# knight46/Quantum_compute_DFT

Measured on AMD Instinct MI355X. Metric: grid_points_per_sec, higher is better.
Workload: dtype f64; 1 GPU; benzene_gga_def2svp: DFT_ComputeXC (GGA) nao=114 ngrid=143556 per GPU, synthetic AO/grid (SURVEY 8(d) recipe), inputs resident in HBM; functional=GGA, nao=114, nocc=21, ngrid_per_gpu=143556, entry_point=DFT_ComputeXC (the reference ABI: full density matrix)

## Files before the change

### include/dft_solver.h

```cpp
#ifndef QCDFT_AMD_DFT_SOLVER_H
#define QCDFT_AMD_DFT_SOLVER_H

#ifdef __cplusplus
extern "C" {
#endif

typedef struct XCSolver XCSolver;

enum SolverType { SOLVER_LDA = 0, SOLVER_GGA = 1, SOLVER_B3LYP = 2,
                  SOLVER_MIX = 3  };

enum XCComponent { XC_SLATER_X = 0, XC_VWN5_C, XC_VWN_RPA_C, XC_PW92_C,
                   XC_PBE_X, XC_PBE_C, XC_B88_X, XC_LYP_C, XC_NCOMP };


XCSolver *DFT_CreateSolver(int type);

void DFT_DestroySolver(XCSolver *solver);

double DFT_ComputeXC(XCSolver *solver, int ngrid, int nao,
                     unsigned long long d_dm_ptr,
                     unsigned long long d_ao_ptr,
                     unsigned long long d_ao_grad_ptr,
                     unsigned long long d_weights_ptr,
// ... 108 lines not shown
int DFT_PointCoulombSetStream(void *handle, unsigned long long hip_stream);
const char *DFT_PointCoulombLastError(void *handle);
void DFT_PointCoulombClose(void *handle);

void *DFT_ScfTailOpen(int nao, int nocc, unsigned long long d_hcore, unsigned long long d_overlap, unsigned long long d_basis,
                      unsigned long long d_fock_out, unsigned long long d_mo_energy);
int DFT_ScfTailSetStream(void *handle, unsigned long long hip_stream);
int DFT_ScfTailStep(void *handle, int rotate, double c_hf, double tol, double canon_tol, int max_inner, int slot, int nhist,
                    const int *hist, const double *coef, unsigned long long d_J, unsigned long long d_K,
                    unsigned long long d_vraw, unsigned long long d_dm, unsigned long long d_cocc, unsigned long long d_exc);
int DFT_ScfTailFinish(void *handle, double c_hf, unsigned long long d_J, unsigned long long d_K, unsigned long long d_dm,
                      unsigned long long d_cocc);
int DFT_ScfTailMore(void *handle, int nsteps, unsigned long long d_J, unsigned long long d_K, unsigned long long d_dm,
                    unsigned long long d_cocc, unsigned long long d_exc);
int DFT_ScfTailSetStepsHint(void *handle, int nsteps);
int DFT_ScfTailWait(void *handle, double *out8);
int DFT_ScfTailGram(void *handle, double *host_out64);
int DFT_ScfTailStamps(void *handle, long long *host_out16);
const char *DFT_ScfTailLastError(void *handle);
void DFT_ScfTailClose(void *handle);

int DFT_SetOption(XCSolver *solver, const char *key, double value);

int DFT_SetStream(XCSolver *solver, unsigned long long hip_stream);

const char *DFT_GetLastError(XCSolver *solver);

int DFT_GetTimings(XCSolver *solver, double *ms, const char **names, int max_entries);

#ifdef __cplusplus
}
#endif
#endif
```

### quantum_compute_dft_amd/build.py

```python
import contextlib
import fcntl
import hashlib
import json
import os
import re
import shutil
import subprocess

PKG_DIR = os.path.dirname(os.path.abspath(__file__))
CSRC = os.path.join(PKG_DIR, "csrc")
LIB_DIR = os.path.join(PKG_DIR, "lib")
LIB_PATH = os.path.join(LIB_DIR, "libdft.so")
STAMP_PATH = LIB_PATH + ".srchash"
SOURCES = ["dft_api.hip", "xc_occ.hip", "eri_cols.hip", "scf_tail.hip", "xc_tiny.hip", "point_coulomb.hip"]
HEADERS = ["xc_functionals.hpp", "xc_kernels.hpp", "xc_ws_kernels.hpp", "xc_big_kernels.hpp",
           "xc_occ_kernels.hpp", "xc_occ_launch.hpp", "xc_tiny_kernels.hpp", "xc_tiny_launch.hpp", "jk_kernels.hpp", "ao_kernels.hpp", "cd_kernels.hpp", "device_util.hpp", "md_device.hpp",
           os.path.join("..", "..", "include", "dft_solver.h")]
FLAGS = ["--offload-arch=gfx950", "-O3", "-std=c++17", "-fPIC",
         "-mllvm", "-amdgpu-mfma-vgpr-form", "-Wall", "-Wno-unused-function"]
EXTRA_FLAGS = {"xc_tiny.hip": ["-mllvm", "-disable-machine-licm"]}
RESOURCES_PATH = LIB_PATH + ".resources.json"

VALIDATION_KERNELS = ("k_rho_mfma", "k_vxc_mfma", "k_rho_valu", "k_vxc_valu")
SPILL_ALLOW = {
    "void qcdft::k_vxc_ws<8, true, false, false>": (8, "one dword (the thread index) stored before and reloaded after the step loop, "
                                                       "never inside it (ISA checked); the 8-byte-load GGA variant for odd nao / "
                                                       "unaligned planes at nao 113-128 only"),
}


def parse_resource_usage(text):
    out = {}
    for blk in re.split(r"remark: Function Name: ", text)[1:]:
        name = blk.split()[0]
        def g(key):
            m = re.search(key + r": (\d+)", blk)
            return int(m.group(1)) if m else 0
        out[name] = {"vgprs": g(r"  VGPRs"), "agprs": g("AGPRs"), "sgprs": g(r"  SGPRs"), "vgpr_spill": g("VGPRs Spill"),
                     "sgpr_spill": g("SGPRs Spill"), "scratch": g(r"ScratchSize \[bytes/lane\]"),
                     "occupancy": g(r"Occupancy \[waves/SIMD\]"), "lds": g(r"LDS Size \[bytes/block\]")}
    return out


def check_spills(res):
    bad = []
    for name, r in sorted(res.items()):
        if not (r["vgpr_spill"] or r["scratch"]):
            continue
# ... 105 lines not shown
```

### quantum_compute_dft_amd/csrc/dft_api.hip

```cpp
#include <hip/hip_runtime.h>

#include <cmath>
#include <cstdarg>
#include <cstdio>
#include <cstdint>
#include <cstdlib>
#include <cstring>
#include <algorithm>
#include <limits>
#include <string>
#include <type_traits>
#include <vector>

#include "../../include/dft_solver.h"
#include "ao_kernels.hpp"
#include "jk_kernels.hpp"
#include "cd_kernels.hpp"
#include "xc_big_kernels.hpp"
#include "xc_ws_kernels.hpp"
#include "xc_kernels.hpp"
#include "xc_occ_launch.hpp"
#include "xc_tiny_launch.hpp"

using namespace qcdft;
// ... 20 lines not shown
    unsigned long stamp = 0;
};

}

struct XCSolver {
    int type = 0;
    bool needs_grad = false;
    xc::MixWeights mix = {};
    hipStream_t stream = nullptr;
    bool device_ok = false;
    int device = 0;
    int num_cu = 256;
    int quirks = 1;
    int path = 0;
    int profile = 0;
    int ksplit = 0;
    int ao_pt = 0;
    int fuse_finish = 0;
    int sweep_order = 2;
    int tiny = -1;
    int occ = 0;
    int used_occ = 0;
    int eri_sym = 0;
    int graph = -1;
    std::vector<SweepGraph> graphs;
    hipStream_t cap_stream = nullptr;
    unsigned long graph_clock = 0, graph_gen = 0;
    DevBuf dsym, rho, sigma, grad, coef, partial, slabs, exc, jpart, kpart, shells, msym, cdy, cdc, cdv, ao_ws, vtmp, occ_cp, occ_dm;
    int spin_wait = 1;
    int strict_sync = 0;
    double *h_exc = nullptr;
    double *h_exc_dev = nullptr;
    std::string last_error;
    std::vector<Timing> timings;
    size_t n_timed = 0;
    std::vector<unsigned char> shell_blob;
};

namespace {

void set_error(XCSolver *s, const char *fmt, ...)
{
    char buf[512];
    va_list ap;
    va_start(ap, fmt);
    vsnprintf(buf, sizeof buf, fmt, ap);
    va_end(ap);
    fprintf(stderr, "libdft: %s\n", buf);
    if (s) s->last_error = buf;
}

bool hip_ok(XCSolver *s, hipError_t e, const char *what)
{
    if (e == hipSuccess) return true;
    set_error(s, "%s failed: %s", what, hipGetErrorString(e));
// ... 73 lines not shown

template <int NT = 1, class F>
void with_nt(int nt, F &&f)
{
    if constexpr (NT < 8) {
        if (nt != NT) return with_nt<NT + 1>(nt, f);
    }
    f(std::integral_constant<int, NT>{});
}

template <class F>
void with_bool(bool b, F &&f)
{
    if (b) f(std::true_type{});
    else   f(std::false_type{});
}

bool xc_sweep(XCSolver *s, long ngrid, int nao, const double *dm, const double *ao,
              const double *ao_grad, const double *w, double *vxc, bool want_host_exc,
              const double *cocc = nullptr, int nocc = 0, double *exc_out = nullptr)
{
    s->last_error.clear();
    s->n_timed = 0;
    if (!s->device_ok) {
        set_error(s, "no usable HIP device");
        return false;
    }
    if (ngrid <= 0 || nao <= 0) {
        set_error(s, "bad sizes ngrid=%ld nao=%d", ngrid, nao);
        return false;
    }
    const bool gga = s->needs_grad;
    if (gga && !ao_grad) {
        set_error(s, "ao_grad pointer is null for a gradient-corrected functional");
        return false;
    }
    if (!dm && !cocc) {
        set_error(s, "neither a density matrix nor occupied orbitals were given");
        return false;
    }
    if (cocc && nocc <= 0) {
        set_error(s, "occupied orbitals given with nocc=%d", nocc);
        return false;
    }
    const bool tiny = s->path == 0 && s->tiny != 0 && s->type != SOLVER_MIX && nao <= TINY_MAX_NAO && (double)ngrid * nao * 8.0 < 4294967296.0 &&
                      (s->tiny > 0 || tiny_pays(s->num_cu, s->type == SOLVER_LDA ? 0 : s->type == SOLVER_GGA ? 1 : 2, nao, ngrid));
// ... 93 lines not shown
                    hipLaunchKernelGGL((k_rho_ws<NT, G, V>), dim3((unsigned)nslab), dim3(WS_THREADS), 0, st, ngrid, nao, ao, gx, gy, gz, dm, rho, grad, sigma, s->sweep_order & 1);
                }); });
            else if (big)
                with_bool(vec16, [&](auto V) {
                    hipLaunchKernelGGL((k_rho_big64<G, V>), dim3((unsigned)((ngrid + R6_BM - 1) / R6_BM)), dim3(256), 0, st, ngrid, nao, NP, ao, gx, gy, gz, Dp, rho, grad, sigma);
                });
            else if (s->path != 1)
                hipLaunchKernelGGL(k_rho_mfma<G>, dim3((unsigned)((ngrid + 63) / 64)), dim3(256), 0, st, ngrid, nao, NP, ao, gx, gy, gz, Dp, rho, grad, sigma);
            else
                hipLaunchKernelGGL(k_rho_valu<G>, dim3((unsigned)((ngrid + 3) / 4)), dim3(256), 0, st, ngrid, nao, NP, ao, gx, gy, gz, Dp, rho, grad, sigma);
        });
    }
    if (!tiny) {
        ScopedTimer t(s, "xc_points");
        dim3 g((unsigned)nxb);
        if (s->type == SOLVER_LDA)      hipLaunchKernelGGL(k_xc_points<0>, g, dim3(256), 0, st, ngrid, rho, sigma, grad, w, coef, partial, s->quirks);
        else if (s->type == SOLVER_GGA) hipLaunchKernelGGL(k_xc_points<1>, g, dim3(256), 0, st, ngrid, rho, sigma, grad, w, coef, partial, s->quirks);
        else if (s->type == SOLVER_B3LYP) hipLaunchKernelGGL(k_xc_points<2>, g, dim3(256), 0, st, ngrid, rho, sigma, grad, w, coef, partial, s->quirks);
        else if (gga)                   hipLaunchKernelGGL(k_xc_points_mix<true>, g, dim3(256), 0, st, ngrid, rho, sigma, grad, w, coef, partial, s->quirks, s->mix);
        else                            hipLaunchKernelGGL(k_xc_points_mix<false>, g, dim3(256), 0, st, ngrid, rho, sigma, grad, w, coef, partial, s->quirks, s->mix);
    }
    if (!tiny) {
        ScopedTimer t(s, "vxc");
        auto launch = [&](auto G, auto S) {
            if (fast)
                with_bool(vec16, [&](auto V) { with_nt(ntv, [&](auto NT) {
                    hipLaunchKernelGGL((k_vxc_ws<NT, G, V, S>), dim3((unsigned)nslab), dim3(WS_THREADS), 0, st, ngrid, nao, ao, gx, gy, gz, coef, slabs, (s->sweep_order >> 1) & 1);
                }); });
            else if (big)
                with_bool(vec16, [&](auto V) {
                    hipLaunchKernelGGL((k_vxc_big<G, V>), dim3((unsigned)(nslab * npair)), dim3(BG_THREADS), 0, st, ngrid, nao, chunk, nB, npair, ao, gx, gy, gz, coef, slabs);
                });
            else if (s->path != 1)
                hipLaunchKernelGGL(k_vxc_mfma<G>, dim3((unsigned)nslab, nblk, nblk), dim3(256), 0, st, ngrid, nao, chunk, ao, gx, gy, gz, coef, slabs);
            else
                hipLaunchKernelGGL(k_vxc_valu<G>, dim3((unsigned)nslab), dim3(256), 0, st, ngrid, nao, chunk, ao, gx, gy, gz, coef, slabs);
        };
        switch (s->type) {
        case SOLVER_LDA: launch(std::false_type{}, std::false_type{}); break;
        case SOLVER_GGA: launch(std::true_type{}, std::false_type{}); break;
        case SOLVER_MIX:
            if (gga) launch(std::true_type{}, std::false_type{});
            else     launch(std::false_type{}, std::false_type{});
            break;
        default:         launch(std::true_type{}, std::true_type{}); break;
        }
    }
    {
        ScopedTimer t(s, "reduce_vxc");
        dim3 g((unsigned)(((size_t)nao * nao + 31) / 32));
        const bool b3 = s->type == SOLVER_B3LYP;
        if (b3 && big) {
            if (!reserve(s, s->msym, sizeof(double) * (size_t)nao * nao, "hipMalloc(M)")) return false;
            double *M = (double *)s->msym.p;
            hipLaunchKernelGGL(k_reduce_slabs8<false>, g, dim3(256), 0, st, nao, nslab, slabs, M);
            const int nt = (nao + 31) / 32;
            hipLaunchKernelGGL(k_symmetrize, dim3((unsigned)(nt * (nt + 1) / 2)), dim3(256), 0, st, nao, M, vxc);
        } else if (b3 && !fast) {
            hipLaunchKernelGGL(k_reduce_slabs8<true>, g, dim3(256), 0, st, nao, nslab, slabs, vxc);
        } else if (s->fuse_finish) {
            hipLaunchKernelGGL((k_reduce_slabs8<false, true>), g, dim3(256), 0, st, nao, nslab, slabs, vxc, nxb, partial, exc,
                               want_host_exc ? s->h_exc_dev : nullptr);
            return hip_ok(s, hipGetLastError(), "XC sweep launch");
        } else {
            hipLaunchKernelGGL((k_reduce_slabs8<false, true>), g, dim3(256), 0, st, nao, nslab, slabs, vxc, nxb, partial, exc, (double *)nullptr);
            if (want_host_exc && s->h_exc_dev) hipLaunchKernelGGL(k_publish_exc, dim3(1), dim3(1), 0, st, exc, s->h_exc_dev);
            return hip_ok(s, hipGetLastError(), "XC sweep launch");
        }
        hipLaunchKernelGGL(k_finish_exc, dim3(1), dim3(256), 0, st, nxb, partial, exc, want_host_exc ? s->h_exc_dev : nullptr);
    }
    return hip_ok(s, hipGetLastError(), "XC sweep launch");
}

void jk(XCSolver *s, int nao, const double *eri, const double *dm, double *J, double *K, int i0 = 0, int ni = -1)
{
    s->last_error.clear();
    if (!s->device_ok) { set_error(s, "no usable HIP device"); return; }
    if (nao <= 0 || nao > JK_COLS) { set_error(s, "dense-ERI J/K needs 1 <= nao <= %d (got %d)", JK_COLS, nao); return; }
    if (ni < 0) ni = nao;
    if (i0 < 0 || ni <= 0 || i0 + ni > nao) { set_error(s, "dense-ERI J/K: bad row range [%d, %d) of %d", i0, i0 + ni, nao); return; }
    if (!J && !K) return;
    const int n = nao;
    const size_t N2 = (size_t)n * n;
    const int KB = std::max(1, std::min(n, JK_COLS / n));
    const int ncb = (n + KB - 1) / KB;
    if (J && !K && s->eri_sym == 2 && i0 == 0 && ni == n && n >= 48) {
        const size_t NPK = (size_t)n * (n + 1) / 2;
        const int nchunk = (int)((NPK + JS8_RC - 1) / JS8_RC);
        int cpt = 4;
// ... 245 lines not shown

void launch_ao(XCSolver *s, const AoTable &t, long ngrid, int nao, const double *coords, double *ao, double *ao_grad)
{
    const bool vec = t.even_blocks && (nao % 2 == 0) && ((uintptr_t)ao % 16 == 0) && ((uintptr_t)ao_grad % 16 == 0);
    const int ao_pt = s->ao_pt ? s->ao_pt : ((ao_grad ? 4 : 1) * 16 * (t.maxcol | 1) * 8 > 53 * 1024 ? 8 : 16);
    launch_eval_ao(s->stream, ngrid, nao, t.nchunk, t.maxcol, vec, ao_pt, s->num_cu, t.nshell, t.nprim, t.sh, t.exp, t.coef, t.chunks, t.order,
                   coords, ao, ao_grad);
}

__global__ void k_accumulate_chunk(long n2, int add, const double *__restrict__ vc, const double *__restrict__ ec,
                                   double *__restrict__ v, double *__restrict__ e)
{
    const long i = (long)blockIdx.x * 256 + threadIdx.x;
    if (i < n2) v[i] = add ? v[i] + vc[i] : vc[i];
    if (i == 0) *e = add ? *e + *ec : *ec;
}

}

extern "C" {

int DFT_GetVersion(void) { return 5; }

static XCSolver *create_solver(int type, const double *mix)
{
    XCSolver *s = new (std::nothrow) XCSolver();
    if (!s) return nullptr;
    s->type = type;
    s->needs_grad = type != SOLVER_LDA;
    if (mix) {
        s->needs_grad = false;
        for (int k = 0; k < XC_NCOMP; ++k) {
            s->mix.c[k] = mix[k];
            if (k >= XC_PBE_X && mix[k] != 0.0) s->needs_grad = true;
        }
    }
    int ndev = 0;
    if (hipGetDeviceCount(&ndev) == hipSuccess && ndev > 0) {
        int dev = 0;
        hipDeviceProp_t prop;
        if (hipGetDevice(&dev) == hipSuccess && hipGetDeviceProperties(&prop, dev) == hipSuccess) {
            s->device_ok = true;
            s->device = dev;
            s->num_cu = prop.multiProcessorCount > 0 ? prop.multiProcessorCount : 256;
        }
        if (s->device_ok) {
            if (hipHostMalloc((void **)&s->h_exc, sizeof(double), hipHostMallocMapped | hipHostMallocCoherent) != hipSuccess ||
                hipHostGetDevicePointer((void **)&s->h_exc_dev, s->h_exc, 0) != hipSuccess) {
                (void)hipGetLastError();
                s->h_exc = nullptr;
                s->h_exc_dev = nullptr;
            }
        }
    } else {
        (void)hipGetLastError();
        s->last_error = "no usable HIP device";
    }
    return s;
}

XCSolver *DFT_CreateSolver(int type)
{
    if (type != SOLVER_LDA && type != SOLVER_GGA && type != SOLVER_B3LYP) return nullptr;
    return create_solver(type, nullptr);
}

XCSolver *DFT_CreateSolverMix(const double *weights, int ncomp)
{
    if (!weights || ncomp != XC_NCOMP) return nullptr;
    bool any = false;
    for (int k = 0; k < XC_NCOMP; ++k) {
        if (!std::isfinite(weights[k])) return nullptr;
        any = any || weights[k] != 0.0;
    }
    if (!any) return nullptr;
// ... 10 lines not shown
    case SOLVER_B3LYP:
        weights_out[XC_SLATER_X] = 0.80; weights_out[XC_B88_X] = 0.72; weights_out[XC_VWN_RPA_C] = 0.19; weights_out[XC_LYP_C] = 0.81;
        break;
    default:
        for (int k = 0; k < XC_NCOMP; ++k) weights_out[k] = s->mix.c[k];
    }
    return 0;
}

void DFT_DestroySolver(XCSolver *s)
{
    if (!s) return;
    if (s->device_ok) {
        DeviceGuard dg(s);
        (void)hipStreamSynchronize(s->stream);
        drop_graphs(s);
        if (s->cap_stream) (void)hipStreamDestroy(s->cap_stream);
        DevBuf *bufs[] = {&s->dsym, &s->rho, &s->sigma, &s->grad, &s->coef, &s->partial,
                          &s->slabs, &s->exc, &s->jpart, &s->kpart, &s->shells, &s->msym,
                          &s->cdy, &s->cdc, &s->cdv, &s->ao_ws, &s->vtmp, &s->occ_cp, &s->occ_dm};
        for (DevBuf *b : bufs)
            if (b->p) (void)hipFree(b->p);
        if (s->h_exc) (void)hipHostFree(s->h_exc);
        for (Timing &t : s->timings) {
            (void)hipEventDestroy(t.t0);
            (void)hipEventDestroy(t.t1);
        }
    }
    delete s;
}

constexpr double GRAPH_AUTO_ELEMS = 2.0e6;

struct SweepArgs {
    long ngrid;
    int nao, nocc;
    const double *dm, *ao, *grad, *w;
    double *vxc;
    const double *cocc;
};

static SweepGraph *find_sweep(XCSolver *s, const SweepArgs &a)
{
    for (SweepGraph &g : s->graphs)
        if (g.ngrid == a.ngrid && g.nao == a.nao && g.nocc == a.nocc && g.dm == a.dm && g.ao == a.ao && g.grad == a.grad &&
            g.w == a.w && g.vxc == a.vxc && g.cocc == a.cocc)
            return &g;
    return nullptr;
}

static bool record_sweep(XCSolver *s, const SweepArgs &a)
{
    if (!s->cap_stream && hipStreamCreateWithFlags(&s->cap_stream, hipStreamNonBlocking) != hipSuccess) {
        (void)hipGetLastError();
        return false;
    }
    const unsigned long gen = s->graph_gen;
    if (hipStreamBeginCapture(s->cap_stream, hipStreamCaptureModeThreadLocal) != hipSuccess) {
        (void)hipGetLastError();
        return false;
    }
    hipStream_t user = s->stream;
    s->stream = s->cap_stream;
    const bool ok = xc_sweep(s, a.ngrid, a.nao, a.dm, a.ao, a.grad, a.w, a.vxc, true, a.cocc, a.nocc);
    s->stream = user;
    hipGraph_t graph = nullptr;
    const hipError_t e = hipStreamEndCapture(s->cap_stream, &graph);
    hipGraphExec_t exec = nullptr;
    const bool good = ok && e == hipSuccess && graph && gen == s->graph_gen &&
                      hipGraphInstantiate(&exec, graph, nullptr, nullptr, 0) == hipSuccess;
    if (graph) (void)hipGraphDestroy(graph);
    if (!good) (void)hipGetLastError();
    SweepGraph *g = gen == s->graph_gen ? find_sweep(s, a) : nullptr;
    if (!g) {
        if (exec) (void)hipGraphExecDestroy(exec);
        return false;
    }
    g->exec = good ? exec : nullptr;
    g->bad = !good;
    return good;
}

static bool replay_sweep(XCSolver *s, const SweepArgs &a)
{
    SweepGraph *g = find_sweep(s, a);
    if (!g || g->bad) return false;
    if (!g->exec && !record_sweep(s, a)) return false;
// ... 26 lines not shown
        s->graphs.erase(s->graphs.begin() + (long)old);
    }
    SweepGraph g;
    g.ngrid = a.ngrid; g.nao = a.nao; g.nocc = a.nocc;
    g.dm = a.dm; g.ao = a.ao; g.grad = a.grad; g.w = a.w; g.vxc = a.vxc; g.cocc = a.cocc;
    g.seen = 1;
    g.stamp = ++s->graph_clock;
    s->graphs.push_back(g);
}

static double xc_call_sync(XCSolver *s, long long ngrid, int nao, unsigned long long d_dm,
                           unsigned long long d_ao, unsigned long long d_ao_grad,
                           unsigned long long d_w, unsigned long long d_vxc,
                           unsigned long long d_cocc, int nocc)
{
    if (!s) return 0.0;
    DeviceGuard dg(s);
    const double nan = std::numeric_limits<double>::quiet_NaN();
    if (s->h_exc) *s->h_exc = nan;
    const SweepArgs a{(long)ngrid, nao, nocc, (const double *)d_dm, (const double *)d_ao, (const double *)d_ao_grad,
                      (const double *)d_w, (double *)d_vxc, (const double *)d_cocc};
    const bool graphed = !s->profile && s->h_exc_dev && ngrid > 0 && nao > 0 &&
                         (s->graph > 0 || (s->graph < 0 && (double)ngrid * nao <= GRAPH_AUTO_ELEMS));
    if (!(graphed && replay_sweep(s, a)) &&
        !xc_sweep(s, a.ngrid, nao, a.dm, a.ao, a.grad, a.w, a.vxc, true, a.cocc, nocc))
        return nan;
    if (graphed) note_sweep(s, a);
    if (s->h_exc_dev) {
        volatile double *hx = s->h_exc;
        if (s->spin_wait) {
            for (unsigned spins = 1; std::isnan(*hx); ++spins) {
                if ((spins & 0xFFF) == 0 && hipStreamQuery(s->stream) != hipErrorNotReady) break;
                __builtin_ia32_pause();
            }
            if (s->strict_sync || std::isnan(*hx)) {
                hipError_t q;
                while ((q = hipStreamQuery(s->stream)) == hipErrorNotReady) __builtin_ia32_pause();
                if (!hip_ok(s, q, "XC sweep")) return nan;
            }
        } else if (!hip_ok(s, hipStreamSynchronize(s->stream), "synchronise")) {
            return nan;
        }
        const double out = *hx;
        if (std::isnan(out)) set_error(s, "Exc is NaN after the sweep completed (non-finite inputs, or the finishing kernel did not run)");
        return out;
    }
    double out = nan;
    if (!hip_ok(s, hipMemcpyAsync(&out, s->exc.p, sizeof(double), hipMemcpyDeviceToHost, s->stream), "copy Exc") ||
        !hip_ok(s, hipStreamSynchronize(s->stream), "synchronise"))
        return nan;
    if (std::isnan(out)) set_error(s, "Exc is NaN after the sweep completed (non-finite inputs)");
    return out;
}
// ... 143 lines not shown
        hipLaunchKernelGGL(k_accumulate_chunk, dim3(nb), dim3(256), 0, s->stream, (long)nao * nao, g0 == 0 ? 0 : 1, vt,
                           (const double *)s->exc.p, (double *)d_vxc, eacc);
    }
    if (d_exc && !hip_ok(s, hipMemcpyAsync((void *)d_exc, eacc, sizeof(double), hipMemcpyDeviceToDevice, s->stream), "copy Exc"))
        return -1;
    return hip_ok(s, hipGetLastError(), "direct XC sweep launch") ? 0 : -1;
}

int DFT_SetOption(XCSolver *s, const char *key, double value)
{
    if (!s || !key) return -1;
    if (strcmp(key, "profile") && strcmp(key, "spin_wait") && strcmp(key, "strict_sync")) {
        DeviceGuard dg(s);
        drop_graphs(s);
    }
    if (!strcmp(key, "eri_symmetric")) { s->eri_sym = value == 2.0 ? 2 : value != 0.0; return 0; }
    if (!strcmp(key, "graph")) { s->graph = value > 0.0 ? 1 : value < 0.0 ? -1 : 0; return 0; }
    if (!strcmp(key, "quirks")) { s->quirks = value != 0.0; return 0; }
    if (!strcmp(key, "path")) { s->path = (int)value; return 0; }
    if (!strcmp(key, "profile")) { s->profile = value != 0.0; return 0; }
    if (!strcmp(key, "spin_wait")) { s->spin_wait = value != 0.0; return 0; }
    if (!strcmp(key, "strict_sync")) { s->strict_sync = value != 0.0; return 0; }
    if (!strcmp(key, "fuse_finish")) { s->fuse_finish = value != 0.0; return 0; }
    if (!strcmp(key, "sweep_order")) { s->sweep_order = (int)value & 3; return 0; }
    if (!strcmp(key, "occ")) { s->occ = value == 1.0 ? 1 : value == 2.0 ? 2 : 0; return 0; }
    if (!strcmp(key, "tiny")) { s->tiny = value > 0.0 ? 1 : value < 0.0 ? -1 : 0; return 0; }
    if (!strcmp(key, "ao_pt")) { s->ao_pt = value == 16.0 ? 16 : value == 8.0 ? 8 : 0; return 0; }
    if (!strcmp(key, "ksplit")) { s->ksplit = value > 0 ? (int)value : 0; return 0; }
    return -1;
}

int DFT_SetStream(XCSolver *s, unsigned long long hip_stream)
{
    if (!s) return -1;
    DeviceGuard dg(s);
    if (s->device_ok) (void)hipStreamSynchronize(s->stream);
    s->stream = (hipStream_t)hip_stream;
    return 0;
}

const char *DFT_GetLastError(XCSolver *s)
{
    return s ? s->last_error.c_str() : "";
}

int DFT_GetTimings(XCSolver *s, double *ms, const char **names, int max_entries)
{
    if (!s || !s->device_ok) return 0;
    DeviceGuard dg(s);
    (void)hipStreamSynchronize(s->stream);
    int n = 0;
    for (size_t i = 0; i < s->n_timed && n < max_entries; ++i, ++n) {
// ... 10 lines not shown
```

### quantum_compute_dft_amd/csrc/xc_ws_kernels.hpp

```cpp
#pragma once
#include <hip/hip_runtime.h>
#include "xc_kernels.hpp"

namespace qcdft {

#ifdef QCDFT_STAMPS
__device__ unsigned long long g_stamps[256 * 8 * 4];
#define QCDFT_T(var) unsigned long long var = __builtin_amdgcn_s_memtime()
#define QCDFT_ACC(slot, a, b) st_acc[slot] += (b) - (a)
#else
#define QCDFT_T(var)
#define QCDFT_ACC(slot, a, b)
#endif

constexpr int WS_ROWS = 16;
constexpr int WS_THREADS = 512;
constexpr int WS_RING = 4;
constexpr int WS_OT = 16;

template <int NT> struct WsCfg {
    static constexpr int NCOL = 16 * NT;
    static constexpr int JN = (NT + 1) / 2;
    static constexpr int LDA = NCOL + 2;
    static constexpr int LDX = ((NCOL + 31) / 32) * 32 + 16;
};

__device__ __forceinline__ unsigned ws_tile(unsigned ntile, unsigned b, unsigned s, unsigned nwg, int rev)
{
    const unsigned t = b + s * nwg;
    return rev ? ntile - 1u - t : t;
}

template <int NT, bool GRAD, bool VEC, bool SYM>
__global__ __launch_bounds__(WS_THREADS, 2) void k_vxc_ws(long ngrid, int nao,
                                                          const double *__restrict__ ao,
                                                          const double *__restrict__ gx,
                                                          const double *__restrict__ gy,
                                                          const double *__restrict__ gz,
                                                          const double *__restrict__ coef,
                                                          double *__restrict__ slabs, int rev)
{
    using C = WsCfg<NT>;
    constexpr int TILE = WS_ROWS * C::LDX;
    constexpr int NTW = (NT + 1) / 2;
    __shared__ double ring[2 * WS_RING * TILE];
    double *const Ps = ring, *const Qs = ring + WS_RING * TILE;

    const int tid = threadIdx.x;
    const int wave = __builtin_amdgcn_readfirstlane(tid >> 6);
    const long ntile = (ngrid + WS_ROWS - 1) / WS_ROWS;
    const long nloc = (ntile > (long)blockIdx.x) ? (ntile - blockIdx.x + gridDim.x - 1) / gridDim.x : 0;
    const long nstep = nloc + 2;

    if (wave < 4) {
        const int lane = tid & 63, li = lane & 15, lk = lane >> 4;
        const int wa = wave >> 1, wb = wave & 1;
        const int na = (NT - wa + 1) / 2, nb = (NT - wb + 1) / 2;
        d4 acc[NTW][NTW];
#pragma unroll
        for (int i = 0; i < NTW; ++i)
#pragma unroll
            for (int j = 0; j < NTW; ++j) acc[i][j] = (d4){0.0, 0.0, 0.0, 0.0};

#ifdef QCDFT_STAMPS
        unsigned long long st_acc[4] = {0, 0, 0, 0};
#endif
        const int fo = lk * C::LDX + li;
        double af[NTW], bf[NTW];
        auto load_frags = [&](int slot, int ks, double (&a_)[NTW], double (&b_)[NTW]) {
            const double *P = Ps + slot * TILE + fo + 4 * ks * C::LDX;
            const double *Q = Qs + slot * TILE + fo + 4 * ks * C::LDX;
#pragma unroll
            for (int i = 0; i < NTW; ++i) {
                a_[i] = Q[16 * min(wa + 2 * i, NT - 1)];
                b_[i] = P[16 * min(wb + 2 * i, NT - 1)];
            }
        };
// ... 39 lines not shown
                for (int j = 0; j < NTW; ++j) {
                    if (i >= na || j >= nb) continue;
                    const int b = 16 * (wb + 2 * j) + li;
#pragma unroll
                    for (int r = 0; r < 4; ++r) {
                        const int a = 16 * (wa + 2 * i) + lk + 4 * r;
                        if (a < nao && b < nao) slab[(size_t)a * nao + b] = acc[i][j][r];
                    }
                }
        } else {
            constexpr int LDM = C::NCOL + 1;
            static_assert(LDM * C::NCOL <= 2 * WS_RING * TILE, "M tile must fit in the ring");
            double *M = ring;
#pragma unroll
            for (int i = 0; i < NTW; ++i)
#pragma unroll
                for (int j = 0; j < NTW; ++j) {
                    if (i >= na || j >= nb) continue;
                    const int b = 16 * (wb + 2 * j) + li;
#pragma unroll
                    for (int r = 0; r < 4; ++r) M[(16 * (wa + 2 * i) + lk + 4 * r) * LDM + b] = acc[i][j][r];
                }
        }
    } else {
        __builtin_amdgcn_s_setprio(3);
        const int lt = tid - 256, row = lt >> 4, seg = lt & 15;
        const double *c0 = coef, *c1 = coef + (size_t)ngrid, *c2 = coef + 2 * (size_t)ngrid,
                     *c3 = coef + 3 * (size_t)ngrid;
        double p0[2][2 * C::JN], p1[2][2 * C::JN], p2[2][2 * C::JN], p3[2][2 * C::JN];
        double k0[2], k1[2], k2[2], k3[2];

        const long plane = ngrid * (long)nao;
        const unsigned voff = (unsigned)(row * nao + 2 * seg) * 8u, koff = (unsigned)row * 8u;
        const unsigned tile_b = (unsigned)(WS_ROWS * nao) * 8u, ktile_b = WS_ROWS * 8u;
        const unsigned plane_b = (unsigned)(plane * 8), coef_b = (unsigned)(ngrid * 8);
        const __amdgpu_buffer_rsrc_t r0 = plane_rsrc(ao, plane), r1 = plane_rsrc(GRAD ? gx : ao, plane),
                                     r2 = plane_rsrc(GRAD ? gy : ao, plane), r3 = plane_rsrc(GRAD ? gz : ao, plane),
                                     q0 = plane_rsrc(c0, ngrid), q1 = plane_rsrc(GRAD ? c1 : c0, ngrid),
                                     q2 = plane_rsrc(GRAD ? c2 : c0, ngrid), q3 = plane_rsrc(GRAD ? c3 : c0, ngrid);
        auto issue = [&](int set, unsigned s) {
            const bool live = s < (unsigned)nloc;
            const unsigned t = ws_tile((unsigned)ntile, blockIdx.x, s, gridDim.x, rev);
            const unsigned so = live ? t * tile_b : plane_b, ko = live ? t * ktile_b : coef_b;
            k0[set] = buf_load_f64(q0, koff, ko);
            if (GRAD) {
                k1[set] = buf_load_f64(q1, koff, ko);
                k2[set] = buf_load_f64(q2, koff, ko);
// ... 392 lines not shown
```

### quantum_compute_dft_amd/solver.py

```python
import ctypes
import os

from . import functionals
from .build import LIB_PATH

_u64 = ctypes.c_uint64


def default_library_path():
    return LIB_PATH


def load_library(lib_path=None):
    try:
        import torch
    except ImportError:
        pass
    return ctypes.CDLL(os.path.abspath(lib_path or default_library_path()))


def _ptr(a):
    if a is None:
        return 0
    if isinstance(a, int):
# ... 41 lines not shown
                                       _u64, _u64, _u64, _u64, _u64, _u64]
        L.DFT_ComputeXCOcc.restype = ctypes.c_double
        L.DFT_ComputeXCOccAsync.argtypes = [ctypes.c_void_p, ctypes.c_longlong, ctypes.c_int, ctypes.c_int,
                                            _u64, _u64, _u64, _u64, _u64, _u64, _u64]
        L.DFT_ComputeXCOccAsync.restype = ctypes.c_int
        L.DFT_ComputeExchange.argtypes = [ctypes.c_void_p, ctypes.c_int, _u64, _u64, _u64]
        L.DFT_ComputeExchange.restype = None
        L.DFT_ComputeJK.argtypes = [ctypes.c_void_p, ctypes.c_int, _u64, _u64, _u64, _u64]
        L.DFT_ComputeJK.restype = None
        L.DFT_ComputeJKRows.argtypes = [ctypes.c_void_p, ctypes.c_int, ctypes.c_int, ctypes.c_int, _u64, _u64, _u64, _u64]
        L.DFT_ComputeJKRows.restype = ctypes.c_int
        L.DFT_ComputeJKFactorized.argtypes = [ctypes.c_void_p, ctypes.c_int, ctypes.c_int, ctypes.c_int,
                                              _u64, _u64, _u64, _u64, _u64]
        L.DFT_ComputeJKFactorized.restype = ctypes.c_int
        dp, ip = ctypes.POINTER(ctypes.c_double), ctypes.POINTER(ctypes.c_int)
        L.DFT_EvalAO.argtypes = [ctypes.c_void_p, ctypes.c_longlong, ctypes.c_int, ctypes.c_int,
                                 dp, ip, ip, ip, ip, dp, dp, ctypes.c_int, _u64, _u64, _u64]
        L.DFT_EvalAO.restype = ctypes.c_int
        L.DFT_ComputeXCDirect.argtypes = [ctypes.c_void_p, ctypes.c_longlong, ctypes.c_int, ctypes.c_int,
                                          dp, ip, ip, ip, ip, dp, dp, ctypes.c_int, _u64, _u64, _u64, _u64, _u64, ctypes.c_longlong]
        L.DFT_ComputeXCDirect.restype = ctypes.c_int
        L.DFT_SetOption.argtypes = [ctypes.c_void_p, ctypes.c_char_p, ctypes.c_double]
        L.DFT_SetOption.restype = ctypes.c_int
        L.DFT_SetStream.argtypes = [ctypes.c_void_p, _u64]
        L.DFT_SetStream.restype = ctypes.c_int
        L.DFT_GetLastError.argtypes = [ctypes.c_void_p]
        L.DFT_GetLastError.restype = ctypes.c_char_p
        L.DFT_GetTimings.argtypes = [ctypes.c_void_p, dp, ctypes.POINTER(ctypes.c_char_p), ctypes.c_int]
        L.DFT_GetTimings.restype = ctypes.c_int
        L.DFT_GetVersion.argtypes = []
        L.DFT_GetVersion.restype = ctypes.c_int
        L.DFT_CreateSolverMix.argtypes = [dp, ctypes.c_int]
        L.DFT_CreateSolverMix.restype = ctypes.c_void_p
        L.DFT_GetMix.argtypes = [ctypes.c_void_p, dp, ctypes.c_int]
        L.DFT_GetMix.restype = ctypes.c_int

        if self.functional.builtin_type is not None:
            self.solver = L.DFT_CreateSolver(self.functional.builtin_type)
        else:
            self.solver = L.DFT_CreateSolverMix((ctypes.c_double * len(self.weights))(*self.weights), len(self.weights))
        if not self.solver:
            raise RuntimeError("Failed to create C++ DFT Solver instance.")

    def __del__(self):
        if hasattr(self, "lib") and hasattr(self, "solver") and self.solver:
            self.lib.DFT_DestroySolver(self.solver)
# ... 69 lines not shown
    def eval_ao(self, shells, d_coords, ngrid, d_ao, d_ao_grad=None):
        keep, args = self._shell_args(shells)
        rc = self.lib.DFT_EvalAO(self.solver, int(ngrid), *args, _u64(_ptr(d_coords)), _u64(_ptr(d_ao)), _u64(_ptr(d_ao_grad)))
        self._check()
        return rc

    def compute_xc_direct(self, shells, ngrid, d_coords, d_weights, d_dm, d_vxc, d_exc, chunk_points=0):
        keep, args = self._shell_args(shells)
        rc = self.lib.DFT_ComputeXCDirect(self.solver, int(ngrid), *args, _u64(_ptr(d_coords)), _u64(_ptr(d_weights)),
                                          _u64(_ptr(d_dm)), _u64(_ptr(d_vxc)), _u64(_ptr(d_exc)), int(chunk_points))
        self._check()
        return rc

    def mix(self):
        out = (ctypes.c_double * len(functionals.COMPONENTS))()
        if self.lib.DFT_GetMix(self.solver, out, len(out)) != 0:
            raise RuntimeError("DFT_GetMix failed")
        return list(out)

    def set_option(self, key, value):
        if self.lib.DFT_SetOption(self.solver, key.encode(), float(value)) != 0:
            raise KeyError(key)

    def set_stream(self, hip_stream):
        self.lib.DFT_SetStream(self.solver, _u64(int(hip_stream)))

    def last_error(self):
        return (self.lib.DFT_GetLastError(self.solver) or b"").decode()

    def timings(self, max_entries=16):
        ms = (ctypes.c_double * max_entries)()
        names = (ctypes.c_char_p * max_entries)()
        n = self.lib.DFT_GetTimings(self.solver, ms, names, max_entries)
        return [(names[i].decode(), ms[i]) for i in range(n)]

    def _check(self):
        err = self.lib.DFT_GetLastError(self.solver)
        if err:
            raise RuntimeError("libdft: " + err.decode())
```

Measured before the change: 650.3 million grid-points/s.

## Add fringe vxc kernel for nao just past 16-multiples and seq-flag host publish

Adds a k_vxc_ws variant for nao with a small remainder over a multiple of 16 (e.g. 114 = 7*16+2). It computes NT-1 full MFMA tiles across three waves and handles the 1-4 leftover rows and columns with scalar FMAs on a fourth wave, avoiding a whole padded 16-wide tile. It also adds an optional host-publish path where the reduce kernel writes exc directly and a stream write of a sequence number signals completion, so the host spins on that counter. The publish path is off by default, and a GetOption query API is added.

```diff
diff --git a/include/dft_solver.h b/include/dft_solver.h
--- a/include/dft_solver.h
+++ b/include/dft_solver.h
@@ -154,6 +154,8 @@
 
 int DFT_SetOption(XCSolver *solver, const char *key, double value);
 
+double DFT_GetOption(XCSolver *solver, const char *key);
+
 int DFT_SetStream(XCSolver *solver, unsigned long long hip_stream);
 
 const char *DFT_GetLastError(XCSolver *solver);
diff --git a/quantum_compute_dft_amd/build.py b/quantum_compute_dft_amd/build.py
--- a/quantum_compute_dft_amd/build.py
+++ b/quantum_compute_dft_amd/build.py
@@ -23,7 +23,7 @@
 
 VALIDATION_KERNELS = ("k_rho_mfma", "k_vxc_mfma", "k_rho_valu", "k_vxc_valu")
 SPILL_ALLOW = {
-    "void qcdft::k_vxc_ws<8, true, false, false>": (8, "one dword (the thread index) stored before and reloaded after the step loop, "
+    "void qcdft::k_vxc_ws<8, true, false, false, false>": (8, "one dword (the thread index) stored before and reloaded after the step loop, "
                                                        "never inside it (ISA checked); the 8-byte-load GGA variant for odd nao / "
                                                        "unaligned planes at nao 113-128 only"),
 }
diff --git a/quantum_compute_dft_amd/csrc/dft_api.hip b/quantum_compute_dft_amd/csrc/dft_api.hip
--- a/quantum_compute_dft_amd/csrc/dft_api.hip
+++ b/quantum_compute_dft_amd/csrc/dft_api.hip
@@ -66,6 +66,9 @@
     int tiny = -1;
     int occ = 0;
     int used_occ = 0;
+    int vxc_fringe = -1;
+    int used_vxc_fringe = 0;
+    int used_publish = 0;
     int eri_sym = 0;
     int graph = -1;
     std::vector<SweepGraph> graphs;
@@ -76,6 +79,12 @@
     int strict_sync = 0;
     double *h_exc = nullptr;
     double *h_exc_dev = nullptr;
+    int publish = -1;
+    bool publish_ok = false;
+    unsigned long long *h_seq = nullptr, *h_seq_dev = nullptr;
+    unsigned long long seq = 0;
+    bool recording = false;
+    int wait_mode = 0;
     std::string last_error;
     std::vector<Timing> timings;
     size_t n_timed = 0;
@@ -195,6 +204,8 @@
 {
     s->last_error.clear();
     s->n_timed = 0;
+    s->wait_mode = 0;
+    s->used_vxc_fringe = 0;
     if (!s->device_ok) {
         set_error(s, "no usable HIP device");
         return false;
@@ -334,9 +345,17 @@
     }
     if (!tiny) {
         ScopedTimer t(s, "vxc");
+        const bool fringe = fast && s->type != SOLVER_B3LYP && s->vxc_fringe != 0 && nao > 16 && nao % 16 >= 1 && nao % 16 <= 4;
+        s->used_vxc_fringe = fringe;
         auto launch = [&](auto G, auto S) {
             if (fast)
                 with_bool(vec16, [&](auto V) { with_nt(ntv, [&](auto NT) {
+                    if constexpr (NT >= 2 && !S) {
+                        if (fringe) {
+                            hipLaunchKernelGGL((k_vxc_ws<NT, G, V, false, true>), dim3((unsigned)nslab), dim3(WS_THREADS), 0, st, ngrid, nao, ao, gx, gy, gz, coef, slabs, (s->sweep_order >> 1) & 1);
+                            return;
+                        }
+                    }
                     hipLaunchKernelGGL((k_vxc_ws<NT, G, V, S>), dim3((unsigned)nslab), dim3(WS_THREADS), 0, st, ngrid, nao, ao, gx, gy, gz, coef, slabs, (s->sweep_order >> 1) & 1);
                 }); });
             else if (big)
@@ -375,8 +394,21 @@
                                want_host_exc ? s->h_exc_dev : nullptr);
             return hip_ok(s, hipGetLastError(), "XC sweep launch");
         } else {
-            hipLaunchKernelGGL((k_reduce_slabs8<false, true>), g, dim3(256), 0, st, nao, nslab, slabs, vxc, nxb, partial, exc, (double *)nullptr);
-            if (want_host_exc && s->h_exc_dev) hipLaunchKernelGGL(k_publish_exc, dim3(1), dim3(1), 0, st, exc, s->h_exc_dev);
+            const bool sw = want_host_exc && s->h_exc_dev && s->publish > 0 && s->publish_ok && !s->recording;
+            hipLaunchKernelGGL((k_reduce_slabs8<false, true>), g, dim3(256), 0, st, nao, nslab, slabs, vxc, nxb, partial, exc,
+                               sw ? s->h_exc_dev : (double *)nullptr);
+            if (sw) {
+                if (hipStreamWriteValue64(st, s->h_seq_dev, s->seq + 1, 0) == hipSuccess) {
+                    ++s->seq;
+                    s->wait_mode = 1;
+                } else {
+                    (void)hipGetLastError();
+                    s->publish_ok = false;
+                    s->wait_mode = 2;
+                }
+            } else if (want_host_exc && s->h_exc_dev) {
+                hipLaunchKernelGGL(k_publish_exc, dim3(1), dim3(1), 0, st, exc, s->h_exc_dev);
+            }
             return hip_ok(s, hipGetLastError(), "XC sweep launch");
         }
         hipLaunchKernelGGL(k_finish_exc, dim3(1), dim3(256), 0, st, nxb, partial, exc, want_host_exc ? s->h_exc_dev : nullptr);
@@ -668,6 +700,25 @@
 
 int DFT_GetVersion(void) { return 5; }
 
+static void probe_publish(XCSolver *s)
+{
+    if (!s->h_exc_dev) return;
+    if (hipHostMalloc((void **)&s->h_seq, sizeof(unsigned long long), hipHostMallocMapped | hipHostMallocCoherent) != hipSuccess ||
+        hipHostGetDevicePointer((void **)&s->h_seq_dev, s->h_seq, 0) != hipSuccess) {
+        (void)hipGetLastError();
+        if (s->h_seq) (void)hipHostFree(s->h_seq);
+        s->h_seq = s->h_seq_dev = nullptr;
+        return;
+    }
+    *s->h_seq = 0;
+    s->seq = 1;
+    if (hipStreamWriteValue64(s->stream, s->h_seq_dev, s->seq, 0) != hipSuccess || hipStreamSynchronize(s->stream) != hipSuccess) {
+        (void)hipGetLastError();
+        return;
+    }
+    s->publish_ok = *(volatile unsigned long long *)s->h_seq == s->seq;
+}
+
 static XCSolver *create_solver(int type, const double *mix)
 {
     XCSolver *s = new (std::nothrow) XCSolver();
@@ -697,6 +748,7 @@
                 s->h_exc = nullptr;
                 s->h_exc_dev = nullptr;
             }
+            probe_publish(s);
         }
     } else {
         (void)hipGetLastError();
@@ -753,6 +805,7 @@
         for (DevBuf *b : bufs)
             if (b->p) (void)hipFree(b->p);
         if (s->h_exc) (void)hipHostFree(s->h_exc);
+        if (s->h_seq) (void)hipHostFree(s->h_seq);
         for (Timing &t : s->timings) {
             (void)hipEventDestroy(t.t0);
             (void)hipEventDestroy(t.t1);
@@ -793,7 +846,9 @@
     }
     hipStream_t user = s->stream;
     s->stream = s->cap_stream;
+    s->recording = true;
     const bool ok = xc_sweep(s, a.ngrid, a.nao, a.dm, a.ao, a.grad, a.w, a.vxc, true, a.cocc, a.nocc);
+    s->recording = false;
     s->stream = user;
     hipGraph_t graph = nullptr;
     const hipError_t e = hipStreamEndCapture(s->cap_stream, &graph);
@@ -866,13 +921,27 @@
                       (const double *)d_w, (double *)d_vxc, (const double *)d_cocc};
     const bool graphed = !s->profile && s->h_exc_dev && ngrid > 0 && nao > 0 &&
                          (s->graph > 0 || (s->graph < 0 && (double)ngrid * nao <= GRAPH_AUTO_ELEMS));
-    if (!(graphed && replay_sweep(s, a)) &&
-        !xc_sweep(s, a.ngrid, nao, a.dm, a.ao, a.grad, a.w, a.vxc, true, a.cocc, nocc))
+    if (graphed && replay_sweep(s, a)) s->wait_mode = 0;
+    else if (!xc_sweep(s, a.ngrid, nao, a.dm, a.ao, a.grad, a.w, a.vxc, true, a.cocc, nocc))
         return nan;
     if (graphed) note_sweep(s, a);
+    s->used_publish = s->wait_mode == 1;
     if (s->h_exc_dev) {
         volatile double *hx = s->h_exc;
-        if (s->spin_wait) {
+        if (s->spin_wait && s->wait_mode == 1) {
+            volatile unsigned long long *hs = s->h_seq;
+            const unsigned long long want = s->seq;
+            for (unsigned spins = 1; *hs != want; ++spins) {
+                if ((spins & 0xFFF) == 0 && hipStreamQuery(s->stream) != hipErrorNotReady) break;
+                __builtin_ia32_pause();
+            }
+            __atomic_thread_fence(__ATOMIC_ACQUIRE);
+            if (s->strict_sync || *hs != want || std::isnan(*hx)) {
+                hipError_t q;
+                while ((q = hipStreamQuery(s->stream)) == hipErrorNotReady) __builtin_ia32_pause();
+                if (!hip_ok(s, q, "XC sweep")) return nan;
+            }
+        } else if (s->spin_wait && s->wait_mode == 0) {
             for (unsigned spins = 1; std::isnan(*hx); ++spins) {
                 if ((spins & 0xFFF) == 0 && hipStreamQuery(s->stream) != hipErrorNotReady) break;
                 __builtin_ia32_pause();
@@ -1062,12 +1131,35 @@
     if (!strcmp(key, "spin_wait")) { s->spin_wait = value != 0.0; return 0; }
     if (!strcmp(key, "strict_sync")) { s->strict_sync = value != 0.0; return 0; }
     if (!strcmp(key, "fuse_finish")) { s->fuse_finish = value != 0.0; return 0; }
+    if (!strcmp(key, "vxc_fringe")) { s->vxc_fringe = value > 0.0 ? 1 : value < 0.0 ? -1 : 0; return 0; }
+    if (!strcmp(key, "publish")) { s->publish = value > 0.0 ? 1 : value < 0.0 ? -1 : 0; return 0; }
     if (!strcmp(key, "sweep_order")) { s->sweep_order = (int)value & 3; return 0; }
     if (!strcmp(key, "occ")) { s->occ = value == 1.0 ? 1 : value == 2.0 ? 2 : 0; return 0; }
     if (!strcmp(key, "tiny")) { s->tiny = value > 0.0 ? 1 : value < 0.0 ? -1 : 0; return 0; }
     if (!strcmp(key, "ao_pt")) { s->ao_pt = value == 16.0 ? 16 : value == 8.0 ? 8 : 0; return 0; }
     if (!strcmp(key, "ksplit")) { s->ksplit = value > 0 ? (int)value : 0; return 0; }
     return -1;
+}
+
+double DFT_GetOption(XCSolver *s, const char *key)
+{
+    const double unknown = std::numeric_limits<double>::quiet_NaN();
+    if (!s || !key) return unknown;
+    if (!strcmp(key, "publish")) return s->publish;
+    if (!strcmp(key, "publish_probe")) return s->publish_ok ? 1.0 : 0.0;
+    if (!strcmp(key, "publish_live")) return s->publish > 0 && s->publish_ok ? 1.0 : 0.0;
+    if (!strcmp(key, "used_publish")) return s->used_publish;
+    if (!strcmp(key, "vxc_fringe")) return s->vxc_fringe;
+    if (!strcmp(key, "used_vxc_fringe")) return s->used_vxc_fringe;
+    if (!strcmp(key, "fuse_finish")) return s->fuse_finish;
+    if (!strcmp(key, "strict_sync")) return s->strict_sync;
+    if (!strcmp(key, "spin_wait")) return s->spin_wait;
+    if (!strcmp(key, "graph")) return s->graph;
+    if (!strcmp(key, "tiny")) return s->tiny;
+    if (!strcmp(key, "sweep_order")) return s->sweep_order;
+    if (!strcmp(key, "path")) return s->path;
+    if (!strcmp(key, "quirks")) return s->quirks;
+    return unknown;
 }
 
 int DFT_SetStream(XCSolver *s, unsigned long long hip_stream)
diff --git a/quantum_compute_dft_amd/csrc/xc_ws_kernels.hpp b/quantum_compute_dft_amd/csrc/xc_ws_kernels.hpp
--- a/quantum_compute_dft_amd/csrc/xc_ws_kernels.hpp
+++ b/quantum_compute_dft_amd/csrc/xc_ws_kernels.hpp
@@ -31,7 +31,122 @@
     return rev ? ntile - 1u - t : t;
 }
 
-template <int NT, bool GRAD, bool VEC, bool SYM>
+template <int NT, int FP>
+__device__ __forceinline__ void vxc_ws_mfma_fringe(const double *Ps, const double *Qs, int tid, int wave, int nao, long nstep,
+                                                   double *__restrict__ slab)
+{
+    using C = WsCfg<NT>;
+    constexpr int NF = NT - 1, F0 = 16 * NF;
+    constexpr int TILE = WS_ROWS * C::LDX;
+    constexpr int NOPP = F0 + 4 > 64 ? 2 : 1;
+    static_assert(NT >= 2 && F0 + 4 <= 128, "one whole tile at least, two opposite indices per lane at most");
+    const int lane = tid & 63, li = lane & 15, lk = lane >> 4;
+    constexpr bool FRW = FP > 0;
+    constexpr int ROWS = FRW ? (NF > 6 ? 1 : 0) : 2, RA = ROWS ? ROWS : 1, NL = FRW ? 2 * FP : 1;
+    const int nr = FRW || NF >= 6 ? ROWS : min(2, max(0, NF - 2 * wave));
+    d4 acc[RA][NF];
+#pragma unroll
+    for (int i = 0; i < RA; ++i)
+#pragma unroll
+        for (int j = 0; j < NF; ++j) acc[i][j] = (d4){0.0, 0.0, 0.0, 0.0};
+    double fa[NL][NOPP], fb[NL][NOPP];
+#pragma unroll
+    for (int f = 0; f < NL; ++f)
+#pragma unroll
+        for (int j = 0; j < NOPP; ++j) { fa[f][j] = 0.0; fb[f][j] = 0.0; }
+    int opp[NOPP];
+#pragma unroll
+    for (int j = 0; j < NOPP; ++j) opp[j] = min(lane + 64 * j, C::NCOL - 1);
+
+    const int fo = lk * C::LDX + li;
+    double af[RA], bf[NF];
+    auto load_frags = [&](int slot, int ks, double (&a_)[RA], double (&b_)[NF]) {
+        if (ROWS == 0) return;
+        const double *P = Ps + slot * TILE + fo + 4 * ks * C::LDX;
+        const double *Q = Qs + slot * TILE + fo + 4 * ks * C::LDX;
+#pragma unroll
+        for (int i = 0; i < RA; ++i) a_[i] = Q[16 * min(2 * wave + i, NF - 1)];
+#pragma unroll
+        for (int j = 0; j < NF; ++j) b_[j] = P[16 * j];
+    };
+    auto fringe_pair = [&](const double *Pr, const double *Qr, const double (&po)[NOPP], const double (&qo)[NOPP], int f) {
+        const double2 pf = *reinterpret_cast<const double2 *>(&Pr[F0 + f]);
+        const double2 qf = *reinterpret_cast<const double2 *>(&Qr[F0 + f]);
+#pragma unroll
+        for (int j = 0; j < NOPP; ++j) {
+            fa[f][j] += qf.x * po[j];
+            fa[f + 1][j] += qf.y * po[j];
+            fb[f][j] += qo[j] * pf.x;
+            fb[f + 1][j] += qo[j] * pf.y;
+        }
+    };
+#pragma unroll
+    for (int i = 0; i < RA; ++i) af[i] = 0.0;
+#pragma unroll
+    for (int j = 0; j < NF; ++j) bf[j] = 0.0;
+    for (long base = 0; base < nstep; base += WS_RING) {
+#pragma unroll
+        for (int u = 0; u < WS_RING; ++u) {
+            const long step = base + u;
+            if (step >= 2 && step < nstep) {
+                if (step == 2) load_frags((u + 2) % WS_RING, 0, af, bf);
+#pragma unroll
+                for (int ks = 0; ks < WS_ROWS / 4; ++ks) {
+                    double an[RA], bn[NF];
+                    if (ks + 1 < WS_ROWS / 4) load_frags((u + 2) % WS_RING, ks + 1, an, bn);
+                    else                      load_frags((u + 3) % WS_RING, 0, an, bn);
+#pragma unroll
+                    for (int i = 0; i < ROWS; ++i)
+                        if (i < nr) {
+#pragma unroll
+                            for (int j = 0; j < NF; ++j) acc[i][j] = mfma_f64(af[i], bf[j], acc[i][j]);
+                        }
+                    if (FRW) {
+#pragma unroll
+                        for (int kk = 0; kk < 4; ++kk) {
+                            const double *Pr = Ps + ((u + 2) % WS_RING) * TILE + (4 * ks + kk) * C::LDX;
+                            const double *Qr = Qs + ((u + 2) % WS_RING) * TILE + (4 * ks + kk) * C::LDX;
+                            double po[NOPP], qo[NOPP];
+#pragma unroll
+                            for (int j = 0; j < NOPP; ++j) { po[j] = Pr[opp[j]]; qo[j] = Qr[opp[j]]; }
+                            fringe_pair(Pr, Qr, po, qo, 0);
+                            if (FP > 1) fringe_pair(Pr, Qr, po, qo, 2);
+                        }
+                    }
+#pragma unroll
+                    for (int i = 0; i < RA; ++i) af[i] = an[i];
+#pragma unroll
+                    for (int j = 0; j < NF; ++j) bf[j] = bn[j];
+                    __builtin_amdgcn_sched_barrier(0);
+                }
+            }
+            __syncthreads();
+        }
+    }
+#pragma unroll
+    for (int i = 0; i < ROWS; ++i) {
+        if (i >= nr) continue;
+#pragma unroll
+        for (int j = 0; j < NF; ++j)
+#pragma unroll
+            for (int r = 0; r < 4; ++r)
+                slab[(size_t)(16 * (2 * wave + i) + lk + 4 * r) * nao + 16 * j + li] = acc[i][j][r];
+    }
+    if (FRW) {
+#pragma unroll
+        for (int f = 0; f < NL; ++f) {
+            if (F0 + f >= nao) continue;
+#pragma unroll
+            for (int j = 0; j < NOPP; ++j) {
+                const int o = lane + 64 * j;
+                if (o < nao) slab[(size_t)(F0 + f) * nao + o] = fa[f][j];
+                if (o < F0)  slab[(size_t)o * nao + F0 + f] = fb[f][j];
+            }
+        }
+    }
+}
+
+template <int NT, bool GRAD, bool VEC, bool SYM, bool FR = false>
 __global__ __launch_bounds__(WS_THREADS, 2) void k_vxc_ws(long ngrid, int nao,
                                                           const double *__restrict__ ao,
                                                           const double *__restrict__ gx,
@@ -52,7 +167,14 @@
     const long nloc = (ntile > (long)blockIdx.x) ? (ntile - blockIdx.x + gridDim.x - 1) / gridDim.x : 0;
     const long nstep = nloc + 2;
 
-    if (wave < 4) {
+    if constexpr (FR) {
+        static_assert(!FR || !SYM, "the fringe variant writes one-sided slabs");
+        double *slab = slabs + (size_t)blockIdx.x * nao * nao;
+        if (wave < 3)                                 vxc_ws_mfma_fringe<NT, 0>(Ps, Qs, tid, wave, nao, nstep, slab);
+        else if (wave == 3 && nao - 16 * (NT - 1) <= 2) vxc_ws_mfma_fringe<NT, 1>(Ps, Qs, tid, 3, nao, nstep, slab);
+        else if (wave == 3)                           vxc_ws_mfma_fringe<NT, 2>(Ps, Qs, tid, 3, nao, nstep, slab);
+    }
+    if (!FR && wave < 4) {
         const int lane = tid & 63, li = lane & 15, lk = lane >> 4;
         const int wa = wave >> 1, wb = wave & 1;
         const int na = (NT - wa + 1) / 2, nb = (NT - wb + 1) / 2;
@@ -138,7 +260,7 @@
                     for (int r = 0; r < 4; ++r) M[(16 * (wa + 2 * i) + lk + 4 * r) * LDM + b] = acc[i][j][r];
                 }
         }
-    } else {
+    } else if (wave >= 4) {
         __builtin_amdgcn_s_setprio(3);
         const int lt = tid - 256, row = lt >> 4, seg = lt & 15;
         const double *c0 = coef, *c1 = coef + (size_t)ngrid, *c2 = coef + 2 * (size_t)ngrid,
diff --git a/quantum_compute_dft_amd/solver.py b/quantum_compute_dft_amd/solver.py
--- a/quantum_compute_dft_amd/solver.py
+++ b/quantum_compute_dft_amd/solver.py
@@ -87,6 +87,8 @@
         L.DFT_ComputeXCDirect.restype = ctypes.c_int
         L.DFT_SetOption.argtypes = [ctypes.c_void_p, ctypes.c_char_p, ctypes.c_double]
         L.DFT_SetOption.restype = ctypes.c_int
+        L.DFT_GetOption.argtypes = [ctypes.c_void_p, ctypes.c_char_p]
+        L.DFT_GetOption.restype = ctypes.c_double
         L.DFT_SetStream.argtypes = [ctypes.c_void_p, _u64]
         L.DFT_SetStream.restype = ctypes.c_int
         L.DFT_GetLastError.argtypes = [ctypes.c_void_p]
@@ -202,6 +204,12 @@
         if self.lib.DFT_SetOption(self.solver, key.encode(), float(value)) != 0:
             raise KeyError(key)
 
+    def get_option(self, key):
+        v = self.lib.DFT_GetOption(self.solver, key.encode())
+        if v != v:
+            raise KeyError(key)
+        return v
+
     def set_stream(self, hip_stream):
         self.lib.DFT_SetStream(self.solver, _u64(int(hip_stream)))
 
```

Result: faster. 668.1 million grid-points/s, median of 6 (+2.7%).
